# alphacep/vosk-tts

Hardware: AMD Instinct MI355X
Metric: audio_samples_per_sec (higher is better)
Workload: dtype f32

## Files before the change

### vosk_tts_amd/csrc/engine_model.hip.h

```cpp
#pragma once
struct ConvW {
  float* w = nullptr;
  float* w16 = nullptr;
  float* wb = nullptr;
  float* bias = nullptr;
  int M = 0, Mpad = 0, Cin = 0, K = 0, n_sg = 0;
};
struct EncLayerW {
  ConvW qkv, o, f1, f2;
  float *ek = nullptr, *ev = nullptr, *g1 = nullptr, *b1 = nullptr, *g2 = nullptr, *b2 = nullptr;
};
struct EncoderW {
  std::vector<EncLayerW> layers;
  int H = 0, F = 0, K = 0;
  int nh = 0, W = 0;
};
struct DDSW {
  std::vector<float*> sw, sb, g1, b1, g2, b2;
  std::vector<float*> swk[3];
  std::vector<float*> wt;
  std::vector<ConvW> pw;
};
struct ConvFlowW {
  float *pre_w = nullptr, *pre_b = nullptr;
  DDSW dds;
  ConvW proj;
};
struct CouplingW {
  ConvW pre, post;
  EncoderW enc;
  std::vector<ConvW> in_layers, rs_layers;
  std::vector<ConvW> rsx;
  ConvW skip_post;
  ConvW qkv_pre;
  int cond_off = 0;
};
struct MonoW {
  EncoderW enc;
  float *post_w = nullptr, *post_b = nullptr;
};
struct ResBlockW {
  ConvW c1[VITS_MAX_RESD], c2[VITS_MAX_RESD];
  int K = 0;
  int dil[VITS_MAX_RESD] = {0};
};
struct UpW {
  ConvW w;
  int u = 0, Ku = 0, cout = 0, taps = 0, pad_l = 0, halo = 0;
  int shift[8] = {0};
// ... 80 lines not shown

struct vits_session;

struct vits_model {
  bool acoustic = true;
  vits_hparams hp;
  int device = 0;
  std::vector<void*> allocs;
  char* slab = nullptr;
  size_t slab_bytes = 0, slab_used = 0;
  const unsigned char* blob = nullptr;
  size_t blob_bytes = 0;
  uint32_t n_entries = 0;
  const vits_blob_entry* entries = nullptr;
  bool missing = false;

  float *emb = nullptr, *emb_g = nullptr;
  float *cond_W = nullptr, *cond_b = nullptr;
  int cond_rows = 0, cond_enc_off = -1, cond_dp_off = -1, cond_dec_off = -1;
  EncoderW enc_p;
  ConvW enc_proj;
  ConvW bert_proj;
  ConvW dp_pre, dp_proj;
  DDSW dp_dds;
  std::vector<ConvFlowW> cf;
  bool dp_det = false;
  ConvW dp_c1, dp_c2;
  float *dp_n1g = nullptr, *dp_n1b = nullptr, *dp_n2g = nullptr, *dp_n2b = nullptr, *dp_pw = nullptr, *dp_pb = nullptr;
  float *ea_m = nullptr, *ea_logs = nullptr;
  float ea_m_h[2] = {0, 0}, ea_logs_h[2] = {0, 0};
  std::vector<CouplingW> flow;
  std::vector<MonoW> mono;
  ConvW conv_pre, conv_post;
  std::vector<UpW> ups;
  std::vector<ResBlockW> rb;
  float *istft_basis = nullptr, *pqmf = nullptr;
  size_t tail_lds = 0;
  bool use_g = false;
  float* zeros = nullptr;
  int* ps_dbg = nullptr;
  std::mutex pack_mu;
  std::map<std::vector<long long>, const float*> packs;
  int n_cu = 0;
  DecGeom geom;
  int rag_halo = 32;
  std::mutex dn_mu;
// ... 144 lines not shown
      const float* w = r < H ? wq : (r < 2 * H ? wk : wv);
      return w[(size_t)(r % H) * H + ci];
    };
    L.qkv = make_conv(m, 3 * H, H, 1, b3.data(), qkv_src);
    const bool bf3 = hp.conv_precision == 1 && H % 64 == 0 && F % 64 == 0;
    if (bf3) add_bf3_packing(m, L.qkv, qkv_src);
    snprintf(nm, sizeof nm, "%s.attn_layers.%d.conv_o", pfx, i);
    L.o = conv_from(m, nm, H, H, 1, true, true, bf3);
    if (W >= 0) {
      L.ek = upload(m, tget(m, 3, 1, NW, dk, "%s.attn_layers.%d.emb_rel_k", pfx, i), (size_t)NW * dk);
      L.ev = upload(m, tget(m, 3, 1, NW, dk, "%s.attn_layers.%d.emb_rel_v", pfx, i), (size_t)NW * dk);
    }
    snprintf(nm, sizeof nm, "%s.ffn_layers.%d.conv_1", pfx, i);
    L.f1 = conv_from(m, nm, F, H, K, true, true, bf3);
    snprintf(nm, sizeof nm, "%s.ffn_layers.%d.conv_2", pfx, i);
    L.f2 = conv_from(m, nm, H, F, K, true, true, bf3);
    L.g1 = upload(m, tget(m, 1, H, -1, -1, "%s.norm_layers_1.%d.gamma", pfx, i), H);
    L.b1 = upload(m, tget(m, 1, H, -1, -1, "%s.norm_layers_1.%d.beta", pfx, i), H);
    L.g2 = upload(m, tget(m, 1, H, -1, -1, "%s.norm_layers_2.%d.gamma", pfx, i), H);
    L.b2 = upload(m, tget(m, 1, H, -1, -1, "%s.norm_layers_2.%d.beta", pfx, i), H);
  }
}

static void load_dds(vits_model* m, DDSW& D, const char* pfx, int C, int K, int n) {
  char nm[200];
  for (int i = 0; i < n && !m->missing; ++i) {
    D.sw.push_back(upload(m, tget(m, 3, C, 1, K, "%s.convs_sep.%d.weight", pfx, i), (size_t)C * K));
    if (K == 3 && !m->missing) {
      const float* w = tget(m, 3, C, 1, K, "%s.convs_sep.%d.weight", pfx, i);
      for (int k = 0; k < 3; ++k) {
        std::vector<float> t(C);
        for (int c = 0; c < C; ++c) t[c] = w[(size_t)c * 3 + k];
        D.swk[k].push_back(upload(m, t.data(), t.size()));
      }
    }
    D.sb.push_back(upload(m, tget(m, 1, C, -1, -1, "%s.convs_sep.%d.bias", pfx, i), C));
    snprintf(nm, sizeof nm, "%s.convs_1x1.%d", pfx, i);
    D.pw.push_back(conv_from(m, nm, C, C, 1, true));
    {
      const float* w = tget(m, 3, C, C, 1, "%s.weight", nm);
      std::vector<float> t((size_t)C * C);
      if (w && C % 4 == 0) for (int co = 0; co < C; ++co) for (int ci = 0; ci < C; ++ci) t[((size_t)(ci / 4) * C + co) * 4 + (ci & 3)] = w[(size_t)co * C + ci];
      D.wt.push_back(upload(m, t.data(), t.size()));
    }
    D.g1.push_back(upload(m, tget(m, 1, C, -1, -1, "%s.norms_1.%d.gamma", pfx, i), C));
    D.b1.push_back(upload(m, tget(m, 1, C, -1, -1, "%s.norms_1.%d.beta", pfx, i), C));
// ... 203 lines not shown
      m->cond_enc_off = add_cond(tget(m, 2, H, G, -1, "enc_p.encoder.spk_emb_linear.weight"),
                                 tget(m, 1, H, -1, -1, "enc_p.encoder.spk_emb_linear.bias"), H);
    if (m->dp_det)
      m->cond_dp_off = add_cond(tget(m, 3, H, G, 1, "dp.cond.weight"), tget(m, 1, H, -1, -1, "dp.cond.bias"), H);
    else
      m->cond_dp_off = add_cond(tget(m, 3, D, G, 1, "dp.cond.weight"), tget(m, 1, D, -1, -1, "dp.cond.bias"), D);
  }

  char nm[200];
  if (m->dp_det) {
    const int K = hp.dp_kernel_size;
    m->dp_c1 = conv_from(m, "dp.conv_1", D, H, K, true);
    m->dp_c2 = conv_from(m, "dp.conv_2", D, D, K, true);
    m->dp_n1g = upload(m, tget(m, 1, D, -1, -1, "dp.norm_1.gamma"), D);
    m->dp_n1b = upload(m, tget(m, 1, D, -1, -1, "dp.norm_1.beta"), D);
    m->dp_n2g = upload(m, tget(m, 1, D, -1, -1, "dp.norm_2.gamma"), D);
    m->dp_n2b = upload(m, tget(m, 1, D, -1, -1, "dp.norm_2.beta"), D);
    m->dp_pw = upload(m, tget(m, 3, 1, D, 1, "dp.proj.weight"), D);
    m->dp_pb = upload(m, tget(m, 1, 1, -1, -1, "dp.proj.bias"), 1);
    if (m->missing) return VITS_ERR_BLOB;
  } else {
    m->dp_pre = conv_from(m, "dp.pre", D, H, 1, true);
    m->dp_proj = conv_from(m, "dp.proj", D, D, 1, true);
    load_dds(m, m->dp_dds, "dp.convs", D, hp.dp_kernel_size, hp.dp_dds_layers);
    m->cf.resize(hp.dp_n_flows);
    const int P = 3 * hp.dp_num_bins - 1;
    for (int k = 1; k < hp.dp_n_flows && !m->missing; ++k) {
      ConvFlowW& c = m->cf[k];
      c.pre_w = upload(m, tget(m, 3, D, 1, 1, "dp.flows.%d.pre.weight", 2 * k + 1), D);
      c.pre_b = upload(m, tget(m, 1, D, -1, -1, "dp.flows.%d.pre.bias", 2 * k + 1), D);
      snprintf(nm, sizeof nm, "dp.flows.%d.convs", 2 * k + 1);
      load_dds(m, c.dds, nm, D, hp.dp_kernel_size, hp.dp_dds_layers);
      snprintf(nm, sizeof nm, "dp.flows.%d.proj", 2 * k + 1);
      c.proj = conv_from(m, nm, P, D, 1, true);
    }
    {
      const float* em = tget(m, 2, 2, 1, -1, "dp.flows.0.m");
      const float* el = tget(m, 2, 2, 1, -1, "dp.flows.0.logs");
      if (m->missing) return VITS_ERR_BLOB;
      m->ea_m = upload(m, em, 2); m->ea_logs = upload(m, el, 2);
    }
  }

  m->flow.resize(hp.flow_n_flows);
  if (mono) m->mono.resize(hp.flow_n_flows);
  const int K5 = hp.flow_kernel_size, L = hp.flow_wn_layers;
  for (int f = 0; f < hp.flow_n_flows && !m->missing; ++f) {
    CouplingW& c = m->flow[f];
    const int fi = (mono ? 3 : 2) * f;
    snprintf(nm, sizeof nm, "flow.flows.%d.pre", fi);
    c.pre = conv_from(m, nm, H, I / 2, 1, true);
    snprintf(nm, sizeof nm, "flow.flows.%d.pre_transformer", fi);
    if (hp.flow_type == 0) load_encoder(m, c.enc, nm, 1, H, H, K5, 2, hp.window_size);
    else if (hp.flow_type == 1) load_encoder(m, c.enc, nm, 2, I / 2, I / 2, 3, 2, -1);
    for (int i = 0; i < L && !m->missing; ++i) {
      const float* w = tget(m, 3, 2 * H, H, K5, "flow.flows.%d.enc.in_layers.%d.weight", fi, i);
      const float* b = tget(m, 1, 2 * H, -1, -1, "flow.flows.%d.enc.in_layers.%d.bias", fi, i);
// ... 104 lines not shown
```

### vosk_tts_amd/csrc/persist.hip.h

```cpp
#pragma once
#include "conv_small.hip.h"
#include "kernels_misc.hip.h"

typedef unsigned long long ll_t;

#define PS_THREADS 512
#define PS_WAVES 8
#define PS_MAX_STEPS 320
#define PS_MAX_T 512
#define PS_MAXC 256
#define PS_MAXU 8
#define PS_TP 21
#define PS_MAXROW 20
#define PS_DKP 128
#define PS_MKT 12
#define PS_SPIN_LIMIT (1 << 18)
#define PS_ERR_TIMEOUT 8

struct PersistCtl {
  unsigned epoch;
  unsigned done;
  unsigned abort;
  unsigned timeouts;
};

enum { PK_IDLE = 0, PK_MM = 1, PK_DDS = 2, PK_LN = 3, PK_EMB = 4, PK_ATT = 5, PK_MERGE = 6, PK_COUPLE = 7, PK_DUR = 8, PK_EXPAND = 9 };
enum {
  PF_RELU = 1 << 8, PF_INMASK = 1 << 9, PF_OUTMASK = 1 << 10, PF_GATE = 1 << 11, PF_SPLINE = 1 << 12, PF_ZINIT = 1 << 13, PF_LAST = 1 << 14,
  PF_PLAIN_IN = 1 << 15,
  PF_DW = 1 << 16, PF_FIN_LN = 1 << 17, PF_FIN_PRE = 1 << 18,
  PF_LN = 1 << 19,
};

struct alignas(16) PRec {
  int kf, a1, a2, a3;
  unsigned long long p[10];
  int b[8];
};
static_assert(sizeof(PRec) == 128, "PRec is 32 dwords");

struct PProgram {
  int n_steps, T, Tp, P;
  int nb; float bound, inv_sqrt_d;
  const int* len;
  const float* ea_m; const float* ea_logs;
  float* logw;
  int* err;
  const PRec* recs;
  int seg_step, T2, Tp2;
  const ll_t* len2;
  ll_t* logw_cells;
};

struct PCall {
// ... 141 lines not shown
    i1 = i0;
  }
}
__device__ __forceinline__ void ps_prefetch_light(const ps_i4& r, int tid, PsPre& pre) {
  const int kind = PR_I(r, 0) & 0xff;
  const PS_G f32x4* pk = PR_P(const f32x4, r, 9);
  const int row = tid & (kind == PK_ATT ? 511 : 255);
  pre.pk0 = pk[row * 2];
  pre.pk1 = pk[row * 2 + 1];
  const int C = PR_I(r, 1) & 0xffff;
  int i0 = tid & 255; i0 = i0 < C ? i0 : C - 1; i0 = i0 < 0 ? 0 : i0;
  pre.ec0 = PR_P(const float, r, 8)[i0];
}
__device__ __forceinline__ void ps_prefetch(const ps_i4& r, int tid, int wave, int lane, PsPre& pre) {
  const int kf = PR_I(r, 0);
  int i0, i1;
  ps_epi_idx(kf, PR_B(r, 3), PR_B(r, 7), tid, 0, i0, i1);
  const PS_G float* b = PR_P(const float, r, 7);
  const PS_G float* c = PR_P(const float, r, 8);
  pre.eb0 = b[i0]; pre.eb1 = b[i1]; pre.ec0 = c[i0]; pre.ec1 = c[i1];
  ps_load_weights(PR_P(const float, r, 6), PR_B(r, 0) & 0x7f, wave, lane, pre.a);
}

#define PS_REC_READY() asm volatile("" : "+v"(rvB))
#ifdef PS_TRACE
#define PS_STAMP(k) do { if (call.trace && tid0 == 0) call.trace[((long long)rank * PS_MAX_STEPS + s) * 8 + (k)] = __builtin_readcyclecounter(); } while (0)
#else
#define PS_STAMP(k) do { } while (0)
#endif

#define PS_LDS_TILE (3 * 16 * (PS_DKP + 4) + (10 + 12) * (PS_DKP + 4))
#define PS_LDS_MRED (PS_WAVES * 256)
static_assert(PS_LDS_TILE >= PS_MAXC * PS_TP, "operand window does not fit");

__global__ void __launch_bounds__(PS_THREADS) persist_kernel(const PProgram* __restrict__ prog, const PCall call) {
  __shared__ __attribute__((aligned(16))) float tile[PS_LDS_TILE];
  __shared__ __attribute__((aligned(16))) float mred[PS_LDS_MRED];
  __shared__ float hb[32 * 16];
  __shared__ float xs[3 * PS_MAXC];
  __shared__ float red[4 * 16];
  __shared__ __attribute__((aligned(16))) float att_r[PS_WAVES * 256];
  __shared__ float att_p[16 * 17];
  const int tid0 = threadIdx.x;
  const int wave0 = __builtin_amdgcn_readfirstlane(tid0 >> 6);
  const int rank = blockIdx.x, P = gridDim.x;
  const int n_steps = prog->n_steps, seg_step = prog->seg_step;
  int T = prog->T, Tp = prog->Tp;
  const PS_G PRec* recs = (const PS_G PRec*)prog->recs;
  auto load_rec = [&](int s) -> ps_i4 {
    const PS_G ps_i4* p = (const PS_G ps_i4*)(recs + ((size_t)(s < n_steps ? s : n_steps - 1) * P + rank));
    return p[tid0 & 7];
  };
  ps_i4 rvB = load_rec(0);
  PsCtx cx;
  {
    unsigned e = __hip_atomic_load(&call.ctl->epoch, __ATOMIC_RELAXED, __HIP_MEMORY_SCOPE_AGENT) + 1u;
    cx.epoch = __builtin_amdgcn_readfirstlane(e ? e : 1u);
  }
  cx.aborted = 0; cx.spins = 0; cx.ctl = call.ctl;
  {
    const int lim = __builtin_amdgcn_readfirstlane(__hip_atomic_load(call.dbg, __ATOMIC_RELAXED, __HIP_MEMORY_SCOPE_AGENT));
    cx.limit = lim > 0 ? lim : PS_SPIN_LIMIT;
// ... 29 lines not shown
        pending = PS_PENDING(ll_bad(q, epoch));
      } while (ps_again(cx, pending));
      len_raw = __builtin_amdgcn_readfirstlane((int)(unsigned)q);
      T = prog->T2; Tp = prog->Tp2;
    }
    if (kind == PK_IDLE) continue;
    PS_STAMP(0);
    const int L = len_raw < T ? len_raw : T;
    if (kind != PK_MM) {
    ps_prefetch_light(rv, tid, pre);
    __syncthreads();

    if (kind == PK_DDS) {
      const int D = PR_I(rv, 1) & 0xffff, d = PR_I(rv, 1) >> 16, t = PR_I(rv, 2);
      const bool dw = (kf & PF_DW) != 0;
      const float invD = 1.0f / (float)D;
      const PS_G ll_t* xin = PR_P(const ll_t, rv, 0);
      const PS_G ll_t* y2 = (kf & PF_FIN_LN) ? PR_P(const ll_t, rv, 1) : nullptr;
      const PS_G ll_t* zc = (kf & PF_FIN_PRE) ? PR_P(const ll_t, rv, 2) : nullptr;
      PS_G ll_t* xout = PR_P(ll_t, rv, 3);
      PS_G ll_t* bout = PR_P(ll_t, rv, 4);
      const int c = (wave & 3) * 64 + lane, h = wave >> 2;
      const bool cok = c < D;
      {
        if (t >= L) {
          if (h == 1 && cok) {
            ll_store(xout + (long long)t * D + c, 0.f, epoch);
            if (dw) ll_store(bout + (long long)t * D + c, 0.f, epoch);
          }
          PS_STAMP(3);
          continue;
        }
        const int t0 = h ? t : t - d, t1 = t + d;
        const bool n0 = cok && (h ? true : (dw && t0 >= 0)), n1 = cok && !h && dw && t1 < L;
        const int tc0 = t0 < 0 ? 0 : t0, tc1 = t1 < Tp ? t1 : Tp - 1;
        float x0 = 0.f, y0 = 0.f, z0 = 0.f, x1 = 0.f, y1 = 0.f, z1 = 0.f;
        {
          unsigned o0 = (unsigned)(tc0 * D + c) * 8u, o1 = (unsigned)(tc1 * D + c) * 8u, oz0 = (unsigned)tc0 * 8u, oz1 = (unsigned)tc1 * 8u;
          bool pending;
          do {
            asm volatile("" : "+v"(o0), "+v"(o1), "+v"(oz0), "+v"(oz1));
            ll_t qx0 = 0, qy0 = 0, qz0 = 0, qx1 = 0, qy1 = 0, qz1 = 0;
            if (n0) {
              qx0 = ll_load_off(xin, o0);
              if (y2) qy0 = ll_load_off(y2, o0);
              if (zc) qz0 = ll_load_off(zc, oz0);
            }
            if (n1) {
              qx1 = ll_load_off(xin, o1);
              if (y2) qy1 = ll_load_off(y2, o1);
              if (zc) qz1 = ll_load_off(zc, oz1);
            }
            unsigned bad = 0;
            if (n0) bad |= ll_bad(qx0, epoch) | (y2 ? ll_bad(qy0, epoch) : 0u) | (zc ? ll_bad(qz0, epoch) : 0u);
            if (n1) bad |= ll_bad(qx1, epoch) | (y2 ? ll_bad(qy1, epoch) : 0u) | (zc ? ll_bad(qz1, epoch) : 0u);
            x0 = ll_val(qx0); y0 = ll_val(qy0); z0 = ll_val(qz0); x1 = ll_val(qx1); y1 = ll_val(qy1); z1 = ll_val(qz1);
            pending = PS_PENDING(bad);
          } while (ps_again(cx, pending));
        }
        PS_STAMP(1); PS_REC_READY();
        const float par[8] = {pre.pk0[0], pre.pk0[1], pre.pk0[2], pre.pk0[3], pre.pk1[0], pre.pk1[1], pre.pk1[2], pre.pk1[3]};
        if (zc) { x0 = par[0] * z0 + par[1] + x0; x1 = par[0] * z1 + par[1] + x1; }
        if (y2) {
          float m0 = n0 ? y0 : 0.f, m1 = n1 ? y1 : 0.f;
          ps_half_sum2(m0, m1, red, wave, lane);
          m0 *= invD; m1 *= invD;
          const float e0 = y0 - m0, e1 = y1 - m1;
          float q0 = n0 ? e0 * e0 : 0.f, q1 = n1 ? e1 * e1 : 0.f;
          ps_half_sum2(q0, q1, red + 16, wave, lane);
          x0 += PS_GELU(e0 * (1.0f / sqrtf(q0 * invD + 1e-5f)) * par[0] + par[1]);
          x1 += PS_GELU(e1 * (1.0f / sqrtf(q1 * invD + 1e-5f)) * par[0] + par[1]);
        }
        const float xi0 = (n0 && t0 < L) ? x0 : 0.f, xi1 = n1 ? x1 : 0.f;
        if (cok) {
          if (h) { xs[PS_MAXC + c] = xi0; ll_store(xout + (long long)t * D + c, xi0, epoch); }
          else { xs[c] = xi0; xs[2 * PS_MAXC + c] = xi1; }
        }
        if (dw) {
          __syncthreads();
          float v = 0.f;
          if (cok) v = par[2] + par[3] * xs[c] + par[4] * xs[PS_MAXC + c] + par[5] * xs[2 * PS_MAXC + c];
          float m = (cok && h) ? v : 0.f, dummy = 0.f;
          ps_half_sum2(m, dummy, red + 32, wave, lane);
          m *= invD;
          const float e = v - m;
          float q = (cok && h) ? e * e : 0.f;
          ps_half_sum2(q, dummy, red + 48, wave, lane);
          if (cok && h) ll_store(bout + (long long)t * D + c, PS_GELU(e * (1.0f / sqrtf(q * invD + 1e-5f)) * par[6] + par[7]), epoch);
        }
      }
      PS_STAMP(3);
      continue;
    }

    if (kind == PK_MERGE) {
      const int C = PR_I(rv, 1), t = PR_I(rv, 2), dk = PR_I(rv, 3) & 0xff, nh = PR_I(rv, 3) >> 8, dk2 = dk + 2;
      const PS_G ll_t* ap = PR_P(const ll_t, rv, 0);
      PS_G ll_t* out = PR_P(ll_t, rv, 3);
      const int d = (wave & 1) * 64 + lane, hd = wave >> 1;
      const bool ok = d < dk && hd < nh;
      const int nkt = (L + 15) >> 4;
      const long long kstr = PR_B(rv, 0);
      {
        float r = 0.f;
        if (t < L) {
          float M = -3.0e38f, num = 0.f, den = 0.f;
          for (int k0 = 0; k0 < nkt; k0 += PS_MKT) {
            float ov[PS_MKT], mv[PS_MKT], lv[PS_MKT];
            unsigned ob = (unsigned)((t * nh + (hd < nh ? hd : 0)) * dk2) * 8u, od = (unsigned)(d < dk ? d : 0) * 8u;
            bool pending;
            do {
// ... 597 lines not shown
        float e = 0.f;
        if (t < T) e = call.noise ? call.noise[(long long)c * T + t]
                                  : (call.solo ? philox_normal(call.item_seeds ? call.item_seeds[0] : seed, 1, (uint32_t)c, (uint32_t)t)
                                               : philox_normal(seed, 1, (uint32_t)c, (uint32_t)t));
        ll_store(PR_P(ll_t, rv, 5) + (long long)c * Tp + t, e * nsw, epoch);
      }
      if (kf & PF_SPLINE) {
        __syncthreads();
        ll_t zq0 = 0, zq1 = 0;
        if (wave == 0) {
          const int t = n0 + (lane & 15);
          const int x0r = (PR_B(rv, 6) >> 16) & 1;
          const PS_G ll_t* zin = PR_P(const ll_t, rv, 4);
          if (lane < 16 && t < L) {
            zq0 = ll_load_off(zin, (unsigned)(x0r * Tp + t) * 8u);
            zq1 = ll_load_off(zin, (unsigned)((1 - x0r) * Tp + t) * 8u);
          }
        }
        const int nb = prog->nb;
        const float bound = prog->bound, isd = prog->inv_sqrt_d;
        float* sc = mred;
        {
          const int which = wave >> 2, col = 4 * (wave & 3) + (lane >> 4), k = lane & 15;
          const bool kok = k < nb;
          const float u = kok ? hb[(which * nb + k) * 16 + col] * isd : -3.0e38f;
          const float mx = ps_row_max(u);
          const float e = kok ? expf(u - mx) : 0.f;
          const float sum = ps_row_sum(e);
          const float mn = 1e-3f;
          float c = kok ? mn + (1.f - mn * nb) * (e / sum) : 0.f;
          c += ps_row_shr<1>(c);
          c += ps_row_shr<2>(c);
          c += ps_row_shr<4>(c);
          c += ps_row_shr<8>(c);
          float* cdst = sc + which * 17 * 16 + col;
          if (k == 0) cdst[0] = -bound;
          if (kok) cdst[(k + 1) * 16] = k == nb - 1 ? bound : 2.f * bound * c - bound;
        }
        __syncthreads();
        if (wave == 0) {
          const int col = lane & 15, t = n0 + col;
          const int x0r = (PR_B(rv, 6) >> 16) & 1, x1r = 1 - x0r, ea_row = (PR_B(rv, 6) >> 20) & 1;
          const PS_G ll_t* zin = PR_P(const ll_t, rv, 4);
          PS_G ll_t* zout = PR_P(ll_t, rv, 5);
          const bool need = lane < 16 && t < L;
          unsigned o0 = (unsigned)(x0r * Tp + t) * 8u, o1 = (unsigned)(x1r * Tp + t) * 8u;
          float z0 = ll_val(zq0), z1 = ll_val(zq1);
          bool pending = PS_PENDING(need ? (ll_bad(zq0, epoch) | ll_bad(zq1, epoch)) : 0u);
          while (ps_again(cx, pending)) {
            asm volatile("" : "+v"(o0), "+v"(o1));
            ll_t q0 = 0, q1 = 0;
            if (need) { q0 = ll_load_off(zin, o0); q1 = ll_load_off(zin, o1); }
            const unsigned bad = need ? (ll_bad(q0, epoch) | ll_bad(q1, epoch)) : 0u;
            z0 = ll_val(q0); z1 = ll_val(q1);
            pending = PS_PENDING(bad);
          }
          if (lane < 16) {
            float v0 = 0.f, v1 = 0.f;
            if (t < L) {
              v0 = z0;
              v1 = z1;
              const float y = z1;
              if (y >= -bound && y <= bound) {
                const float* cw = sc + col;
                const float* ch = sc + 17 * 16 + col;
                int bin = -1;
                for (int k = 0; k <= nb; ++k) {
                  const float loc = ch[k * 16] + (k == nb ? 1e-6f : 0.f);
                  if (y >= loc) bin++;
                }
                bin = bin < 0 ? 0 : (bin > nb - 1 ? nb - 1 : bin);
                const float in_cw = cw[bin * 16], in_w = cw[(bin + 1) * 16] - in_cw;
                const float in_ch = ch[bin * 16], in_h = ch[(bin + 1) * 16] - in_ch;
                const float min_d = 1e-3f;
                const float cst = spline_cst;
                const float ud0 = (bin == 0) ? cst : hb[(2 * nb + bin - 1) * 16 + col];
                const float ud1 = (bin == nb - 1) ? cst : hb[(2 * nb + bin) * 16 + col];
                const float d0 = min_d + softplus_f(ud0), d1 = min_d + softplus_f(ud1);
                const float delta = in_h / in_w;
                const float t1 = (y - in_ch) * (d0 + d1 - 2.f * delta);
                const float qa = t1 + in_h * (delta - d0);
                const float qb = in_h * d0 - t1;
                const float qc = -delta * (y - in_ch);
                const float disc = qb * qb - 4.f * qa * qc;
                const float root = (2.f * qc) / (-qb - sqrtf(disc));
                v1 = root * in_w + in_cw;
              }
            }
            if (zout) {
              ll_store(zout + (long long)x0r * Tp + t, v0, epoch);
              ll_store(zout + (long long)x1r * Tp + t, v1, epoch);
            }
            if ((kf & PF_LAST) && t < T) {
              const float zz = ea_row == x0r ? v0 : v1;
              const float lw = t < L ? (zz - ea_m) * ea_is : 0.f;
              ((PS_G float*)prog->logw)[t] = lw;
              if (prog->logw_cells) ll_store((PS_G ll_t*)prog->logw_cells + t, lw, epoch);
            }
          }
        }
      }
    }
    PS_STAMP(3);
  }
  __syncthreads();
  if (tid0 == 0) {
    const bool timed_out = cx.aborted || __hip_atomic_load(&call.ctl->abort, __ATOMIC_RELAXED, __HIP_MEMORY_SCOPE_AGENT);
    if (timed_out) atomicOr((int*)prog->err, PS_ERR_TIMEOUT);
    const unsigned old = atomicAdd(&call.ctl->done, 1u);
    if (old == gridDim.x - 1) {
// ... 17 lines not shown
```

### vosk_tts_amd/csrc/persist_plan.hip.h

```cpp
#pragma once

#define PERSIST_SDP 1
#define PERSIST_ENC 2
#define PERSIST_FLOW 4

static int persist_slice(int Cin, int K) {
  if (Cin % 16 || (K != 1 && K != 3 && K != 5)) return 0;
  for (int ks = 1; ks <= 4; ++ks) {
    if (Cin % ks) continue;
    const int cs = Cin / ks;
    if (cs % 16 == 0 && cs <= PS_MAXC && (cs / 16) * K <= PS_MAXU * PS_WAVES) return cs;
  }
  return 0;
}
static bool persist_conv_ok(const ConvW& W) { return W.w16 && persist_slice(W.Cin, W.K) > 0; }

static bool persist_encoder_ok(const vits_model* m, const EncoderW& E) {
  (void)m;
  if (E.layers.empty() || E.H % 16 || E.H > PS_MAXC || E.nh < 1 || E.nh > 4 || E.H % E.nh) return false;
  const int dk = E.H / E.nh;
  if (dk > PS_DKP || dk % 16 || E.W < 1 || E.W > 4 || (2 * E.W + 1) * dk > 1024) return false;
  for (const EncLayerW& L : E.layers)
    if (!persist_conv_ok(L.qkv) || !persist_conv_ok(L.o) || !persist_conv_ok(L.f1) || !persist_conv_ok(L.f2) || L.qkv.K != 1 || L.o.K != 1) return false;
  return true;
// ... 4 lines not shown
  return v < 16 ? 16 : (v > PS_MAX_T ? PS_MAX_T : v);
}
static bool persist_common_ok(const vits_model* m, int B, int T) {
  return m->acoustic && B == 1 && T >= 1 && T <= persist_max_t() && m->n_cu >= 16 && m->zeros;
}

static bool persist_sdp_eligible(const vits_model* m, int B, int Tx) {
  const vits_hparams& hp = m->hp;
  if (m->dp_det) return false;
  if (!persist_common_ok(m, B, Tx)) return false;
  const int D = hp.dp_filter_channels, H = hp.hidden_channels;
  if (D % 32 || D > PS_MAXC || H % 16 || H > PS_MAXC || hp.dp_kernel_size != 3) return false;
  const int nl = (int)m->dp_dds.pw.size();
  if (nl < 1 || nl > 3 || hp.dp_n_flows < 2 || hp.dp_num_bins > 16 || 3 * hp.dp_num_bins - 1 > 32) return false;
  if (1 + 2 * (nl + 1) * hp.dp_n_flows > PS_MAX_STEPS) return false;
  if (!persist_conv_ok(m->dp_pre) || !persist_conv_ok(m->dp_proj) || (int)m->dp_dds.swk[0].size() != nl) return false;
  for (const ConvW& c : m->dp_dds.pw) if (!persist_conv_ok(c)) return false;
  for (int k = 1; k < hp.dp_n_flows; ++k) {
    if ((int)m->cf[k].dds.pw.size() != nl || (int)m->cf[k].dds.swk[0].size() != nl || !persist_conv_ok(m->cf[k].proj)) return false;
    for (const ConvW& c : m->cf[k].dds.pw) if (!persist_conv_ok(c)) return false;
  }
  return true;
}
static size_t persist_sdp_cells(const vits_model* m, int B, int Tx) {
  if (!persist_sdp_eligible(m, B, Tx)) return 0;
  const vits_hparams& hp = m->hp;
  const size_t Tp = (size_t)cdiv(Tx, 16) * 16, D = hp.dp_filter_channels, nl = m->dp_dds.pw.size(), nf = hp.dp_n_flows;
  return Tp * (D * (1 + nf * (3 * nl + 2)) + 2 * (nf + 1));
}

static size_t persist_enc_layer_cells(const vits_model* m, const EncoderW& E, size_t Tp) {
  const size_t H = E.H, F = E.F, nh = E.nh, dk = H / nh, ntn = Tp / 16;
  const size_t ks2 = E.layers[0].f2.Cin / persist_slice(E.layers[0].f2.Cin, E.layers[0].f2.K);
  return Tp * (3 * H + ntn * nh * (dk + 2) + H + H + H + F + ks2 * H + H);
}
static bool persist_enc_eligible(const vits_model* m, int B, int Tx) {
  const vits_hparams& hp = m->hp;
  if (!persist_common_ok(m, B, Tx) || !persist_encoder_ok(m, m->enc_p) || !persist_conv_ok(m->enc_proj) || m->enc_proj.K != 1) return false;
  if (hp.bert_dim > 0 && (!persist_conv_ok(m->bert_proj) || m->bert_proj.K != 1)) return false;
  return 4 + 8 * (int)m->enc_p.layers.size() <= PS_MAX_STEPS;
}
static size_t persist_enc_cells(const vits_model* m, int B, int Tx) {
  if (!persist_enc_eligible(m, B, Tx)) return 0;
  const size_t Tp = (size_t)cdiv(Tx, 16) * 16, H = m->hp.hidden_channels;
  size_t bert = 0;
  if (m->hp.bert_dim > 0) bert = Tp * H * (m->bert_proj.Cin / persist_slice(m->bert_proj.Cin, 1) + 1);
  return Tp * H + bert + m->enc_p.layers.size() * persist_enc_layer_cells(m, m->enc_p, Tp);
}

static bool persist_flow_eligible(const vits_model* m, int B, int Ty) {
  const vits_hparams& hp = m->hp;
// ... 36 lines not shown
  int zinit;
  int blen;
  const float* w16;
  const float* bias;
  const float* cond;
  const ll_t* bin;
  const float* bin_plain;
  const ll_t* res;
  int rpitch;
  ll_t* yout;
  float* yplain;
  const ll_t* z;
  ll_t* zout;
  int z_row;
  int last, ea_row;
  int C, plen;
  int padd[8];
  const float* par[8];
  const float* vec;
  int dil, dw, fin;
  const ll_t* xin; const ll_t* y2;
  ll_t* xout;
  ll_t* bout;
  int np, ln;
  const ll_t* part; long long part_stride;
  const ll_t* base;
  const float* emb; float scale; int n_vocab;
  int nh, dk, W;
  const ll_t* qkv;
  ll_t* ap;
  const float* ek; const float* ev;
  const ll_t* u; const float* u_plain;
  int H;
  ll_t* out;
  float* oplain;
};

static const float* persist_pack(vits_session* s, const float* const (&src)[8], const int (&add)[8], int len, int rows) {
  vits_model* m = s->m;
  std::vector<long long> key;
  for (int k = 0; k < 8; ++k) { key.push_back((long long)(uintptr_t)src[k]); key.push_back(add[k]); }
  key.push_back(len); key.push_back(rows);
  for (auto& pk : s->ps_pending)
    if (pk.first == key) return pk.second;
  float* dst = nullptr;
  {
// ... 244 lines not shown
        (void)src;
        pack = persist_pack(s, sk, add, (2 * st.W + 1) * st.dk, 512);
        if (!pack) { bad = true; return; }
      }
      for (int i0 = 0; i0 < items; i0 += P) {
        PRec* R = new_step();
        for (int item = i0; item < std::min(items, i0 + P); ++item) {
          const int kt = item % ntn, qt = (item / ntn) % ntn, hd = item / (ntn * ntn);
          PRec& r = R[item - i0];
          r.kf = PK_ATT;
          r.a1 = st.dk | (st.nh << 8) | (st.W << 16);
          r.a2 = (qt * 16) | ((kt * 16) << 16);
          r.a3 = hd | (kt << 8);
          r.p[0] = U(st.qkv); r.p[1] = U(st.ap); r.p[9] = U(pack);
        }
      }
    } else {
      PRec* R = nullptr;
      const float* pack = m->zeros;
      if (st.kind != PK_MERGE && st.kind != PK_EMB) {
        pack = persist_pack(s, st.par, st.padd, st.plen, 256);
        if (!pack) { bad = true; return; }
      }
      for (int t = 0; t < Tp; ++t) {
        if (t % P == 0) R = new_step();
        PRec& r = R[t % P];
        r.a1 = st.C; r.a2 = t; r.p[9] = U(pack);
        r.p[3] = U(st.out); r.p[4] = U(st.oplain);
        r.b[4] = st.plain_T;
        if (st.kind == PK_DDS) {
          r.kf = PK_DDS | (st.dw ? PF_DW : 0) | (st.fin == 1 ? PF_FIN_LN : 0) | (st.fin == 2 ? PF_FIN_PRE : 0);
          r.a1 = st.C | (st.dil << 16);
          r.p[0] = U(st.xin); r.p[1] = U(st.y2); r.p[2] = st.z ? U(st.z + (size_t)st.z_row * Tp) : 0; r.p[3] = U(st.xout); r.p[4] = U(st.bout);
        } else if (st.kind == PK_LN) {
          r.kf = PK_LN | (st.ln ? PF_LN : 0);
          r.a3 = st.np;
          r.p[0] = U(st.part); r.p[1] = U(st.res); r.p[2] = U(st.base);
          r.p[8] = U(st.vec ? st.vec : m->zeros);
          r.b[0] = (int)(unsigned)(st.part_stride & 0xffffffffll); r.b[1] = (int)(st.part_stride >> 32);
        } else if (st.kind == PK_EMB) {
          r.kf = PK_EMB;
          r.p[0] = U(st.emb);
          r.p[8] = U(st.vec ? st.vec : m->zeros);
          memcpy(&r.b[0], &st.scale, 4);
          r.b[1] = st.n_vocab;
        } else if (st.kind == PK_MERGE) {
          r.kf = PK_MERGE;
          r.a3 = st.dk | (st.nh << 8);
          r.p[0] = U(st.ap);
          r.b[0] = Tp * st.nh * (st.dk + 2);
        } else {
          r.kf = PK_COUPLE | (st.u_plain ? PF_PLAIN_IN : 0);
          r.a3 = st.np | (st.H << 16);
          r.p[0] = U(st.part); r.p[1] = U(st.u); r.p[2] = U(st.u_plain);
          r.b[0] = (int)(unsigned)(st.part_stride & 0xffffffffll); r.b[1] = (int)(st.part_stride >> 32);
        }
// ... 82 lines not shown
    x = persist_encoder_layer(b, m->enc_p.layers[i], m->enc_p, x, (i + 1 == cond_layer) ? vec : nullptr, nullptr, i == n - 1 ? s->x : nullptr);
  st = b.mm(m->enc_proj, x, H);
  st.in_mask = 1; st.out_mask = 1;
  st.yplain = s->stats;
  st.yout = stats_cells;
  b.push(st);
  return x;
}

static void seg_sdp(vits_session* s, PBuild& b, const ll_t* x_cells) {
  vits_model* m = s->m;
  const vits_hparams& hp = m->hp;
  std::vector<PStep>& steps = *b.steps;
  const int D = hp.dp_filter_channels, nl = (int)m->dp_dds.pw.size(), K = hp.dp_kernel_size, H = hp.hidden_channels;
  PStep st = b.mm(m->dp_pre, x_cells, H);
  if (!x_cells) st.bin_plain = s->x;
  if (m->use_g && m->cond_dp_off >= 0) st.cond = s->condv + m->cond_dp_off;
  st.zinit = 1;
  st.yout = b.take_rows(D); st.zout = b.take_rows(2);
  if (x_cells && !steps.empty() && steps.back().kind == PK_MM && steps.back().Tp == b.Tp) { st.join = 1; b.fit_pair(steps.back(), st); }
  const size_t first = steps.size();
  const ll_t* x = b.push(st).yout;
  const ll_t* z = steps[first].zout;
  auto stack = [&](const DDSW& Wd, const ConvW& proj, bool spline, const ll_t* xin, const ll_t* zc, int z_row, const float* pw, const float* pb) -> PStep& {
    const ll_t* y2 = nullptr;
    int dil = 1;
    for (int i = 0; i <= nl; ++i) {
      const bool fin = i == nl;
      st = b.blank(PK_DDS);
      st.C = D; st.plen = D; st.dw = fin ? 0 : 1; st.dil = fin ? 0 : dil;
      st.xin = xin; st.y2 = y2;
      if (i > 0) { st.fin = 1; st.par[0] = Wd.g2[i - 1]; st.par[1] = Wd.b2[i - 1]; }
      else if (zc) { st.fin = 2; st.z = zc; st.z_row = z_row; st.par[0] = pw; st.par[1] = pb; }
      if (!fin) {
        st.par[2] = Wd.sb[i]; st.par[3] = Wd.swk[0][i]; st.par[4] = Wd.swk[1][i]; st.par[5] = Wd.swk[2][i];
        st.par[6] = Wd.g1[i]; st.par[7] = Wd.b1[i];
        st.bout = b.take_rows(D);
      }
      st.xout = b.take_rows(D);
      b.flops += 2.0 * b.T * (double)D * (fin ? 0 : K);
      const PStep& col = b.push(st);
      xin = col.xout;
      st = b.mm(fin ? proj : Wd.pw[i], fin ? col.xout : col.bout, D);
      if (fin) {
        if (spline) { st.epi = PS_EPI_SPLINE; st.mbg = st.n_mb; st.G = 1; }
        else st.out_mask = 1;
        return b.push(st);
      }
      st.yout = b.take_rows(D);
      y2 = b.push(st).yout;
      dil *= K;
    }
    return steps[first];
  };
  {
    PStep& pj = stack(m->dp_dds, m->dp_proj, false, x, nullptr, 0, nullptr, nullptr);
    pj.yout = b.take_rows(D);
  }
  const ll_t* dc = steps.back().yout;
  int swap = 0;
  for (int k = hp.dp_n_flows - 1; k >= 1; --k) {
    swap ^= 1;
    const ConvFlowW& c = m->cf[k];
    PStep& pj = stack(c.dds, c.proj, true, dc, z, swap, c.pre_w, c.pre_b);
    pj.z = z; pj.z_row = swap;
    if (k > 1) { pj.zout = b.take_rows(2); z = pj.zout; }
    else { pj.last = 1; pj.ea_row = swap ^ 1; }
  }
}

static void seg_flow(vits_session* s, PBuild& b, const ll_t* zp_cells) {
  vits_model* m = s->m;
  const vits_hparams& hp = m->hp;
  const int H = hp.hidden_channels, I = hp.inter_channels, half = I / 2, L = hp.flow_wn_layers;
  const ll_t* u = zp_cells;
  for (int f = hp.flow_n_flows - 1; f >= 0; --f) {
    const CouplingW& C = m->flow[f];
    PStep st = b.mm(C.pre, u, I, I - 1, -1);
    if (!u) st.bin_plain = s->zA;
    st.out_mask = 1;
    st.yout = b.take_rows(H);
    const ll_t* fx;
    if (C.qkv_pre.w16 && persist_slice(C.qkv_pre.Cin, 1) == C.qkv_pre.Cin) {
      PStep q = b.mm(C.qkv_pre, u, I, I - 1, -1);
      if (!u) q.bin_plain = s->zA;
      st.join = 1;
      b.fit_pair(q, st);
// ... 145 lines not shown
```

Measured before the change: 45.93 million.

## Fuse SDP 1x1 projections into DDS steps as per-timestep matvecs

In the stochastic duration predictor of the persistent kernel, the separate 1x1 matmul steps (pointwise convs and the final projection) are folded into the preceding depthwise-separable steps. Each timestep's LayerNorm/GELU output stays in shared memory and is multiplied against transposed weights preloaded in registers. Output channels are split across several work items per timestep, and the spline coupling is computed inline for the final projection. This removes intermediate global cell buffers and whole steps with their inter-step synchronisation. In exchange there are more work items per step, duplicated depthwise work across the splits, and extra shape-eligibility constraints.

```diff
diff --git a/vosk_tts_amd/csrc/engine_model.hip.h b/vosk_tts_amd/csrc/engine_model.hip.h
--- a/vosk_tts_amd/csrc/engine_model.hip.h
+++ b/vosk_tts_amd/csrc/engine_model.hip.h
@@ -25,6 +25,7 @@
   float *pre_w = nullptr, *pre_b = nullptr;
   DDSW dds;
   ConvW proj;
+  float* proj_wt = nullptr;
 };
 struct CouplingW {
   ConvW pre, post;
@@ -151,6 +152,7 @@
   ConvW enc_proj;
   ConvW bert_proj;
   ConvW dp_pre, dp_proj;
+  float* dp_proj_wt = nullptr;
   DDSW dp_dds;
   std::vector<ConvFlowW> cf;
   bool dp_det = false;
@@ -341,6 +343,17 @@
   }
 }
 
+static float* conv_wt4(vits_model* m, const char* name, int Cout, int Cin) {
+  const vits_hparams& hp = m->hp;
+  if (Cin % 32 || Cin > PS_MAXC || hp.dp_kernel_size != 3 || hp.dp_dds_layers < 1 || hp.dp_dds_layers > 3 || hp.dp_n_flows < 2) return nullptr;
+  const float* w = tget(m, 3, Cout, Cin, 1, "%s.weight", name);
+  if (!w || m->missing) return nullptr;
+  std::vector<float> t((size_t)Cout * Cin);
+  for (int co = 0; co < Cout; ++co)
+    for (int ci = 0; ci < Cin; ++ci) t[((size_t)(ci / 4) * Cout + co) * 4 + (ci & 3)] = w[(size_t)co * Cin + ci];
+  return upload(m, t.data(), t.size());
+}
+
 static void load_dds(vits_model* m, DDSW& D, const char* pfx, int C, int K, int n) {
   char nm[200];
   for (int i = 0; i < n && !m->missing; ++i) {
@@ -590,6 +603,7 @@
   } else {
     m->dp_pre = conv_from(m, "dp.pre", D, H, 1, true);
     m->dp_proj = conv_from(m, "dp.proj", D, D, 1, true);
+    m->dp_proj_wt = conv_wt4(m, "dp.proj", D, D);
     load_dds(m, m->dp_dds, "dp.convs", D, hp.dp_kernel_size, hp.dp_dds_layers);
     m->cf.resize(hp.dp_n_flows);
     const int P = 3 * hp.dp_num_bins - 1;
@@ -601,6 +615,7 @@
       load_dds(m, c.dds, nm, D, hp.dp_kernel_size, hp.dp_dds_layers);
       snprintf(nm, sizeof nm, "dp.flows.%d.proj", 2 * k + 1);
       c.proj = conv_from(m, nm, P, D, 1, true);
+      c.proj_wt = conv_wt4(m, nm, P, D);
     }
     {
       const float* em = tget(m, 2, 2, 1, -1, "dp.flows.0.m");
diff --git a/vosk_tts_amd/csrc/persist.hip.h b/vosk_tts_amd/csrc/persist.hip.h
--- a/vosk_tts_amd/csrc/persist.hip.h
+++ b/vosk_tts_amd/csrc/persist.hip.h
@@ -30,6 +30,7 @@
   PF_PLAIN_IN = 1 << 15,
   PF_DW = 1 << 16, PF_FIN_LN = 1 << 17, PF_FIN_PRE = 1 << 18,
   PF_LN = 1 << 19,
+  PF_MV = 1 << 20,
 };
 
 struct alignas(16) PRec {
@@ -217,6 +218,74 @@
   ps_load_weights(PR_P(const float, r, 6), PR_B(r, 0) & 0x7f, wave, lane, pre.a);
 }
 
+struct PsMv { f32x4 a[PS_MAXU]; float bias; };
+__device__ __forceinline__ void ps_mv_request(const ps_i4& r, int tid, int wave, int lane, PsMv& pre) {
+  const PS_G char* base = (const PS_G char*)PR_P(const float, r, 6);
+  const int n = PR_B(r, 1), kq = PR_B(r, 3);
+  const unsigned rowb = (unsigned)PR_B(r, 2);
+  const unsigned lane_off = (unsigned)(lane < n ? lane : n - 1) * 16u;
+#pragma unroll
+  for (int i = 0; i < PS_MAXU; ++i) {
+    const unsigned ro = (unsigned)__builtin_amdgcn_readfirstlane(wave * kq + (i < kq ? i : kq - 1)) * rowb;
+    pre.a[i] = *(const PS_G f32x4*)(base + (ro + lane_off));
+  }
+  pre.bias = PR_P(const float, r, 7)[tid < n ? tid : n - 1];
+}
+__device__ __forceinline__ float ps_mv_dot(const PsMv& pre, const float* bcol, int wave, int kq) {
+  const f32x4* b4 = reinterpret_cast<const f32x4*>(bcol) + wave * kq;
+  float acc = 0.f;
+#pragma unroll
+  for (int i = 0; i < PS_MAXU; ++i)
+    if (i < kq) {
+      const f32x4 bb = b4[i];
+      acc = fmaf(pre.a[i][0], bb[0], acc); acc = fmaf(pre.a[i][1], bb[1], acc);
+      acc = fmaf(pre.a[i][2], bb[2], acc); acc = fmaf(pre.a[i][3], bb[3], acc);
+    }
+  return acc;
+}
+
+__device__ __forceinline__ void ps_spline_knots(const float* h, int hs, int which, int k, int nb, float isd, float bound, float* cdst, int cs) {
+  const bool kok = k < nb;
+  const float u = kok ? h[(which * nb + k) * hs] * isd : -3.0e38f;
+  const float mx = ps_row_max(u);
+  const float e = kok ? expf(u - mx) : 0.f;
+  const float sum = ps_row_sum(e);
+  const float mn = 1e-3f;
+  float c = kok ? mn + (1.f - mn * nb) * (e / sum) : 0.f;
+  c += ps_row_shr<1>(c);
+  c += ps_row_shr<2>(c);
+  c += ps_row_shr<4>(c);
+  c += ps_row_shr<8>(c);
+  if (k == 0) cdst[0] = -bound;
+  if (kok) cdst[(k + 1) * cs] = k == nb - 1 ? bound : 2.f * bound * c - bound;
+}
+__device__ __forceinline__ float ps_spline_solve(float y, const float* cw, const float* ch, int cs, const float* hd, int hs, int nb, float bound, float cst) {
+  float v1 = y;
+  if (y >= -bound && y <= bound) {
+    int bin = -1;
+    for (int k = 0; k <= nb; ++k) {
+      const float loc = ch[k * cs] + (k == nb ? 1e-6f : 0.f);
+      if (y >= loc) bin++;
+    }
+    bin = bin < 0 ? 0 : (bin > nb - 1 ? nb - 1 : bin);
+    const float in_cw = cw[bin * cs], in_w = cw[(bin + 1) * cs] - in_cw;
+    const float in_ch = ch[bin * cs], in_h = ch[(bin + 1) * cs] - in_ch;
+    const float min_d = 1e-3f;
+    const float ud0 = (bin == 0) ? cst : hd[(bin - 1) * hs];
+    const float ud1 = (bin == nb - 1) ? cst : hd[bin * hs];
+    const float d0 = min_d + softplus_f(ud0), d1 = min_d + softplus_f(ud1);
+    const float delta = in_h / in_w;
+    const float t1 = (y - in_ch) * (d0 + d1 - 2.f * delta);
+    const float qa = t1 + in_h * (delta - d0);
+    const float qb = in_h * d0 - t1;
+    const float qc = -delta * (y - in_ch);
+    const float disc = qb * qb - 4.f * qa * qc;
+    const float root = (2.f * qc) / (-qb - sqrtf(disc));
+    v1 = root * in_w + in_cw;
+  }
+  return v1;
+}
+
 #define PS_REC_READY() asm volatile("" : "+v"(rvB))
 #ifdef PS_TRACE
 #define PS_STAMP(k) do { if (call.trace && tid0 == 0) call.trace[((long long)rank * PS_MAX_STEPS + s) * 8 + (k)] = __builtin_readcyclecounter(); } while (0)
@@ -232,7 +301,7 @@
   __shared__ __attribute__((aligned(16))) float tile[PS_LDS_TILE];
   __shared__ __attribute__((aligned(16))) float mred[PS_LDS_MRED];
   __shared__ float hb[32 * 16];
-  __shared__ float xs[3 * PS_MAXC];
+  __shared__ __attribute__((aligned(16))) float xs[3 * PS_MAXC];
   __shared__ float red[4 * 16];
   __shared__ __attribute__((aligned(16))) float att_r[PS_WAVES * 256];
   __shared__ float att_p[16 * 17];
@@ -308,11 +377,27 @@
       PS_G ll_t* bout = PR_P(ll_t, rv, 4);
       const int c = (wave & 3) * 64 + lane, h = wave >> 2;
       const bool cok = c < D;
+      const bool mv = (kf & PF_MV) != 0;
+      const int mv_n = PR_B(rv, 1), mv_kq = PR_B(rv, 3);
+      PsMv mvw;
+#pragma unroll
+      for (int i = 0; i < PS_MAXU; ++i) mvw.a[i] = f32x4{0.f, 0.f, 0.f, 0.f};
+      mvw.bias = 0.f;
+      if (mv) ps_mv_request(rv, tid, wave, lane, mvw);
       {
         if (t >= L) {
           if (h == 1 && cok) {
-            ll_store(xout + (long long)t * D + c, 0.f, epoch);
-            if (dw) ll_store(bout + (long long)t * D + c, 0.f, epoch);
+            if (xout) ll_store(xout + (long long)t * D + c, 0.f, epoch);
+            if (dw && !mv) ll_store(bout + (long long)t * D + c, 0.f, epoch);
+          }
+          if (mv && !(kf & PF_SPLINE) && tid < mv_n) ll_store(bout + (long long)t * PR_B(rv, 5) + tid, 0.f, epoch);
+          if ((kf & PF_SPLINE) && tid == 0) {
+            PS_G ll_t* zout = PR_P(ll_t, rv, 2);
+            if (zout) { ll_store(zout + t, 0.f, epoch); ll_store(zout + Tp + t, 0.f, epoch); }
+            if ((kf & PF_LAST) && t < T) {
+              ((PS_G float*)prog->logw)[t] = 0.f;
+              if (prog->logw_cells) ll_store((PS_G ll_t*)prog->logw_cells + t, 0.f, epoch);
+            }
           }
           PS_STAMP(3);
           continue;
@@ -321,12 +406,17 @@
         const bool n0 = cok && (h ? true : (dw && t0 >= 0)), n1 = cok && !h && dw && t1 < L;
         const int tc0 = t0 < 0 ? 0 : t0, tc1 = t1 < Tp ? t1 : Tp - 1;
         float x0 = 0.f, y0 = 0.f, z0 = 0.f, x1 = 0.f, y1 = 0.f, z1 = 0.f;
+        const PS_G ll_t* zs = (kf & PF_SPLINE) ? PR_P(const ll_t, rv, 5) : nullptr;
+        const int x0r = (PR_B(rv, 6) >> 16) & 1;
+        float zs0 = 0.f, zs1 = 0.f;
         {
           unsigned o0 = (unsigned)(tc0 * D + c) * 8u, o1 = (unsigned)(tc1 * D + c) * 8u, oz0 = (unsigned)tc0 * 8u, oz1 = (unsigned)tc1 * 8u;
+          unsigned os0 = (unsigned)(x0r * Tp + t) * 8u, os1 = (unsigned)((1 - x0r) * Tp + t) * 8u;
           bool pending;
           do {
-            asm volatile("" : "+v"(o0), "+v"(o1), "+v"(oz0), "+v"(oz1));
-            ll_t qx0 = 0, qy0 = 0, qz0 = 0, qx1 = 0, qy1 = 0, qz1 = 0;
+            asm volatile("" : "+v"(o0), "+v"(o1), "+v"(oz0), "+v"(oz1), "+v"(os0), "+v"(os1));
+            ll_t qx0 = 0, qy0 = 0, qz0 = 0, qx1 = 0, qy1 = 0, qz1 = 0, qs0 = 0, qs1 = 0;
+            if (zs) { qs0 = ll_load_off(zs, os0); qs1 = ll_load_off(zs, os1); }
             if (n0) {
               qx0 = ll_load_off(xin, o0);
               if (y2) qy0 = ll_load_off(y2, o0);
@@ -340,7 +430,9 @@
             unsigned bad = 0;
             if (n0) bad |= ll_bad(qx0, epoch) | (y2 ? ll_bad(qy0, epoch) : 0u) | (zc ? ll_bad(qz0, epoch) : 0u);
             if (n1) bad |= ll_bad(qx1, epoch) | (y2 ? ll_bad(qy1, epoch) : 0u) | (zc ? ll_bad(qz1, epoch) : 0u);
+            if (zs) bad |= ll_bad(qs0, epoch) | ll_bad(qs1, epoch);
             x0 = ll_val(qx0); y0 = ll_val(qy0); z0 = ll_val(qz0); x1 = ll_val(qx1); y1 = ll_val(qy1); z1 = ll_val(qz1);
+            zs0 = ll_val(qs0); zs1 = ll_val(qs1);
             pending = PS_PENDING(bad);
           } while (ps_again(cx, pending));
         }
@@ -359,7 +451,7 @@
         }
         const float xi0 = (n0 && t0 < L) ? x0 : 0.f, xi1 = n1 ? x1 : 0.f;
         if (cok) {
-          if (h) { xs[PS_MAXC + c] = xi0; ll_store(xout + (long long)t * D + c, xi0, epoch); }
+          if (h) { xs[PS_MAXC + c] = xi0; if (xout) ll_store(xout + (long long)t * D + c, xi0, epoch); }
           else { xs[c] = xi0; xs[2 * PS_MAXC + c] = xi1; }
         }
         if (dw) {
@@ -372,7 +464,44 @@
           const float e = v - m;
           float q = (cok && h) ? e * e : 0.f;
           ps_half_sum2(q, dummy, red + 48, wave, lane);
-          if (cok && h) ll_store(bout + (long long)t * D + c, PS_GELU(e * (1.0f / sqrtf(q * invD + 1e-5f)) * par[6] + par[7]), epoch);
+          const float bv = PS_GELU(e * (1.0f / sqrtf(q * invD + 1e-5f)) * par[6] + par[7]);
+          if (cok && h) { if (mv) xs[c] = bv; else ll_store(bout + (long long)t * D + c, bv, epoch); }
+        }
+        if (mv) {
+          __syncthreads();
+          PS_STAMP(2);
+          mred[wave * 64 + lane] = ps_mv_dot(mvw, dw ? xs : xs + PS_MAXC, wave, mv_kq);
+          __syncthreads();
+          PS_STAMP(4);
+          if (tid < mv_n) {
+            float v = mvw.bias;
+#pragma unroll
+            for (int w = 0; w < PS_WAVES; ++w) v += mred[w * 64 + tid];
+            if (kf & PF_SPLINE) hb[tid] = v;
+            else ll_store(bout + (long long)t * PR_B(rv, 5) + tid, v, epoch);
+          }
+          if (kf & PF_SPLINE) {
+            const int nb = prog->nb;
+            const float bound = prog->bound, isd = prog->inv_sqrt_d;
+            float* sc = mred + PS_WAVES * 64;
+            __syncthreads();
+            if (wave == 0 && lane < 32) ps_spline_knots(hb, 1, lane >> 4, lane & 15, nb, isd, bound, sc + (lane >> 4) * 17, 1);
+            __syncthreads();
+            if (tid == 0) {
+              const int x1r = 1 - x0r, ea_row = (PR_B(rv, 6) >> 20) & 1;
+              PS_G ll_t* zout = PR_P(ll_t, rv, 2);
+              const float v0 = zs0, v1 = ps_spline_solve(zs1, sc, sc + 17, 1, hb + 2 * nb, 1, nb, bound, spline_cst);
+              if (zout) {
+                ll_store(zout + (long long)x0r * Tp + t, v0, epoch);
+                ll_store(zout + (long long)x1r * Tp + t, v1, epoch);
+              }
+              if (kf & PF_LAST) {
+                const float lw = ((ea_row == x0r ? v0 : v1) - ea_m) * ea_is;
+                ((PS_G float*)prog->logw)[t] = lw;
+                if (prog->logw_cells) ll_store((PS_G ll_t*)prog->logw_cells + t, lw, epoch);
+              }
+            }
+          }
         }
       }
       PS_STAMP(3);
@@ -1016,20 +1145,7 @@
         float* sc = mred;
         {
           const int which = wave >> 2, col = 4 * (wave & 3) + (lane >> 4), k = lane & 15;
-          const bool kok = k < nb;
-          const float u = kok ? hb[(which * nb + k) * 16 + col] * isd : -3.0e38f;
-          const float mx = ps_row_max(u);
-          const float e = kok ? expf(u - mx) : 0.f;
-          const float sum = ps_row_sum(e);
-          const float mn = 1e-3f;
-          float c = kok ? mn + (1.f - mn * nb) * (e / sum) : 0.f;
-          c += ps_row_shr<1>(c);
-          c += ps_row_shr<2>(c);
-          c += ps_row_shr<4>(c);
-          c += ps_row_shr<8>(c);
-          float* cdst = sc + which * 17 * 16 + col;
-          if (k == 0) cdst[0] = -bound;
-          if (kok) cdst[(k + 1) * 16] = k == nb - 1 ? bound : 2.f * bound * c - bound;
+          ps_spline_knots(hb + col, 16, which, k, nb, isd, bound, sc + which * 17 * 16 + col, 16);
         }
         __syncthreads();
         if (wave == 0) {
@@ -1053,33 +1169,7 @@
             float v0 = 0.f, v1 = 0.f;
             if (t < L) {
               v0 = z0;
-              v1 = z1;
-              const float y = z1;
-              if (y >= -bound && y <= bound) {
-                const float* cw = sc + col;
-                const float* ch = sc + 17 * 16 + col;
-                int bin = -1;
-                for (int k = 0; k <= nb; ++k) {
-                  const float loc = ch[k * 16] + (k == nb ? 1e-6f : 0.f);
-                  if (y >= loc) bin++;
-                }
-                bin = bin < 0 ? 0 : (bin > nb - 1 ? nb - 1 : bin);
-                const float in_cw = cw[bin * 16], in_w = cw[(bin + 1) * 16] - in_cw;
-                const float in_ch = ch[bin * 16], in_h = ch[(bin + 1) * 16] - in_ch;
-                const float min_d = 1e-3f;
-                const float cst = spline_cst;
-                const float ud0 = (bin == 0) ? cst : hb[(2 * nb + bin - 1) * 16 + col];
-                const float ud1 = (bin == nb - 1) ? cst : hb[(2 * nb + bin) * 16 + col];
-                const float d0 = min_d + softplus_f(ud0), d1 = min_d + softplus_f(ud1);
-                const float delta = in_h / in_w;
-                const float t1 = (y - in_ch) * (d0 + d1 - 2.f * delta);
-                const float qa = t1 + in_h * (delta - d0);
-                const float qb = in_h * d0 - t1;
-                const float qc = -delta * (y - in_ch);
-                const float disc = qb * qb - 4.f * qa * qc;
-                const float root = (2.f * qc) / (-qb - sqrtf(disc));
-                v1 = root * in_w + in_cw;
-              }
+              v1 = ps_spline_solve(z1, sc + col, sc + 17 * 16 + col, 16, hb + 2 * nb * 16 + col, 16, nb, bound, spline_cst);
             }
             if (zout) {
               ll_store(zout + (long long)x0r * Tp + t, v0, epoch);
diff --git a/vosk_tts_amd/csrc/persist_plan.hip.h b/vosk_tts_amd/csrc/persist_plan.hip.h
--- a/vosk_tts_amd/csrc/persist_plan.hip.h
+++ b/vosk_tts_amd/csrc/persist_plan.hip.h
@@ -50,11 +50,24 @@
   }
   return true;
 }
+static int persist_sdp_split(const vits_model* m, int Tx) {
+  const int D = m->hp.dp_filter_channels, Tp = cdiv(Tx, 16) * 16;
+  if (!m->dp_proj_wt || m->dp_dds.wt.size() != m->dp_dds.pw.size() || 3 * m->hp.dp_num_bins - 1 > 64) return 0;
+  for (float* w : m->dp_dds.wt) if (!w) return 0;
+  for (int k = 1; k < m->hp.dp_n_flows; ++k) {
+    if (!m->cf[k].proj_wt) return 0;
+    if (m->cf[k].dds.wt.size() != m->cf[k].dds.pw.size()) return 0;
+    for (float* w : m->cf[k].dds.wt) if (!w) return 0;
+  }
+  const int split = std::min(4, m->n_cu / Tp);
+  return (split >= 1 && cdiv(D, split) <= 64) ? split : 0;
+}
 static size_t persist_sdp_cells(const vits_model* m, int B, int Tx) {
   if (!persist_sdp_eligible(m, B, Tx)) return 0;
   const vits_hparams& hp = m->hp;
   const size_t Tp = (size_t)cdiv(Tx, 16) * 16, D = hp.dp_filter_channels, nl = m->dp_dds.pw.size(), nf = hp.dp_n_flows;
-  return Tp * (D * (1 + nf * (3 * nl + 2)) + 2 * (nf + 1));
+  const size_t per_stack = persist_sdp_split(m, Tx) ? 2 * nl + 1 : 3 * nl + 2;
+  return Tp * (D * (1 + nf * per_stack) + 2 * (nf + 1));
 }
 
 static size_t persist_enc_layer_cells(const vits_model* m, const EncoderW& E, size_t Tp) {
@@ -137,6 +150,8 @@
   const ll_t* xin; const ll_t* y2;
   ll_t* xout;
   ll_t* bout;
+  int mv_split, mv_cout;
+  const float* mv_wt; const float* mv_bias;
   int np, ln;
   const ll_t* part; long long part_stride;
   const ll_t* base;
@@ -427,9 +442,12 @@
         pack = persist_pack(s, st.par, st.padd, st.plen, 256);
         if (!pack) { bad = true; return; }
       }
-      for (int t = 0; t < Tp; ++t) {
-        if (t % P == 0) R = new_step();
-        PRec& r = R[t % P];
+      const int sp = (st.kind == PK_DDS && st.mv_split > 0) ? st.mv_split : 1;
+      if (sp > 1 && Tp * sp > P) { bad = true; return; }
+      for (int item = 0; item < Tp * sp; ++item) {
+        const int t = item / sp, part = item % sp;
+        if (item % P == 0) R = new_step();
+        PRec& r = R[item % P];
         r.a1 = st.C; r.a2 = t; r.p[9] = U(pack);
         r.p[3] = U(st.out); r.p[4] = U(st.oplain);
         r.b[4] = st.plain_T;
@@ -437,6 +455,23 @@
           r.kf = PK_DDS | (st.dw ? PF_DW : 0) | (st.fin == 1 ? PF_FIN_LN : 0) | (st.fin == 2 ? PF_FIN_PRE : 0);
           r.a1 = st.C | (st.dil << 16);
           r.p[0] = U(st.xin); r.p[1] = U(st.y2); r.p[2] = st.z ? U(st.z + (size_t)st.z_row * Tp) : 0; r.p[3] = U(st.xout); r.p[4] = U(st.bout);
+          r.b[1] = 1; r.b[3] = 1;
+          if (st.mv_split > 0) {
+            const int per = cdiv(st.mv_cout, sp), o0 = part * per, n = std::min(per, st.mv_cout - o0);
+            if (n < 1 || per > 64 || st.C % 32 || st.C / 32 > PS_MAXU) { bad = true; return; }
+            r.kf |= PF_MV;
+            if (part > 0) r.p[3] = 0;
+            r.p[4] = U(st.bout + o0);
+            r.p[6] = U(st.mv_wt + (size_t)o0 * 4);
+            r.p[7] = U(st.mv_bias ? st.mv_bias + o0 : m->zeros);
+            r.b[1] = n; r.b[2] = st.mv_cout * 16; r.b[3] = st.C / 32; r.b[5] = st.mv_cout;
+            if (st.epi == PS_EPI_SPLINE) {
+              if (sp != 1 || st.dw) { bad = true; return; }
+              r.kf |= PF_SPLINE | (st.last ? PF_LAST : 0);
+              r.p[2] = U(st.zout); r.p[4] = 0; r.p[5] = U(st.z);
+              r.b[6] = (st.z_row << 16) | (st.ea_row << 20);
+            }
+          }
         } else if (st.kind == PK_LN) {
           r.kf = PK_LN | (st.ln ? PF_LN : 0);
           r.a3 = st.np;
@@ -565,11 +600,13 @@
   const size_t first = steps.size();
   const ll_t* x = b.push(st).yout;
   const ll_t* z = steps[first].zout;
-  auto stack = [&](const DDSW& Wd, const ConvW& proj, bool spline, const ll_t* xin, const ll_t* zc, int z_row, const float* pw, const float* pb) -> PStep& {
+  const int split = persist_sdp_split(m, b.T);
+  auto stack = [&](const DDSW& Wd, const ConvW& proj, const float* proj_wt, bool spline, const ll_t* xin, const ll_t* zc, int z_row, const float* pw, const float* pb) -> PStep& {
     const ll_t* y2 = nullptr;
     int dil = 1;
     for (int i = 0; i <= nl; ++i) {
       const bool fin = i == nl;
+      const bool fused = split > 0;
       st = b.blank(PK_DDS);
       st.C = D; st.plen = D; st.dw = fin ? 0 : 1; st.dil = fin ? 0 : dil;
       st.xin = xin; st.y2 = y2;
@@ -580,8 +617,23 @@
         st.par[6] = Wd.g1[i]; st.par[7] = Wd.b1[i];
         st.bout = b.take_rows(D);
       }
+      b.flops += 2.0 * b.T * (double)D * (fin ? 0 : K);
+      if (fused) {
+        const ConvW& cv = fin ? proj : Wd.pw[i];
+        st.mv_split = split; st.mv_cout = cv.M; st.mv_wt = fin ? proj_wt : Wd.wt[i]; st.mv_bias = cv.bias;
+        b.flops += 2.0 * b.T * (double)cv.M * D;
+        if (fin && spline) {
+          st.bout = nullptr; st.mv_split = 1; st.epi = PS_EPI_SPLINE;
+          return b.push(st);
+        }
+        if (fin) { st.bout = b.take_rows(D); return b.push(st); }
+        st.xout = b.take_rows(D);
+        const PStep& col = b.push(st);
+        xin = col.xout; y2 = col.bout;
+        dil *= K;
+        continue;
+      }
       st.xout = b.take_rows(D);
-      b.flops += 2.0 * b.T * (double)D * (fin ? 0 : K);
       const PStep& col = b.push(st);
       xin = col.xout;
       st = b.mm(fin ? proj : Wd.pw[i], fin ? col.xout : col.bout, D);
@@ -597,15 +649,15 @@
     return steps[first];
   };
   {
-    PStep& pj = stack(m->dp_dds, m->dp_proj, false, x, nullptr, 0, nullptr, nullptr);
-    pj.yout = b.take_rows(D);
-  }
-  const ll_t* dc = steps.back().yout;
+    PStep& pj = stack(m->dp_dds, m->dp_proj, m->dp_proj_wt, false, x, nullptr, 0, nullptr, nullptr);
+    if (pj.kind == PK_MM) pj.yout = b.take_rows(D);
+  }
+  const ll_t* dc = steps.back().kind == PK_MM ? steps.back().yout : steps.back().bout;
   int swap = 0;
   for (int k = hp.dp_n_flows - 1; k >= 1; --k) {
     swap ^= 1;
     const ConvFlowW& c = m->cf[k];
-    PStep& pj = stack(c.dds, c.proj, true, dc, z, swap, c.pre_w, c.pre_b);
+    PStep& pj = stack(c.dds, c.proj, c.proj_wt, true, dc, z, swap, c.pre_w, c.pre_b);
     pj.z = z; pj.z_row = swap;
     if (k > 1) { pj.zout = b.take_rows(2); z = pj.zout; }
     else { pj.last = 1; pj.ea_row = swap ^ 1; }
```

After: 47.87 million (median of 6 runs). 1.04x the previous value.
